# david-zwicker/video-analysis

Measured on AMD Instinct MI355X. Metric: frames/sec (bg-sub+blur+thresh+CCL) 1080p uint8, higher is better.
Workload: dtype u8; 1 GPU; cfg3_1080p_full_chain: 1920x1080 uint8, batch 256/GPU, running-mean bg-sub (f64 state) + sigma=5 Gaussian (q8.8) + threshold 20 + 5x5 dilate/erode + 4-connected labelling + object counts; inputs resident in HBM; engine=bg=1 gauss=mfma-i8(ksize=31) thresh=20 morph=2 ccl=4, video=one clip per rank, overlap=off, world_size=1, backend=single process

## Files before the change

### video-analysis_amd/csrc/va_point.hip

```cpp
#include <math.h>

#include "va_common.h"

namespace va {

namespace {

constexpr int kBlock = 256;
constexpr int kVec = 8;

__device__ __forceinline__ uint8_t sat_u8_trunc(double d)
{
    const int v = (int)d;
    return (uint8_t)(v > 255 ? 255 : v);
}

template <int V>
__global__ void __launch_bounds__(kBlock)
bg_mean_u8_kernel(const uint8_t *__restrict__ frames, uint8_t *__restrict__ diff,
                  double *__restrict__ mean, long long n_seen, int n, size_t px)
{
    size_t i0 = ((size_t)blockIdx.x * kBlock + threadIdx.x) * V;
    if (i0 >= px)
        return;
    double m[V];
#pragma unroll
    for (int k = 0; k < V; k++)
        m[k] = mean[i0 + k];
    for (int f = 0; f < n; f++) {
        uint8_t p[V];
        if (V == 8) {
            uint2 v = *reinterpret_cast<const uint2 *>(frames + (size_t)f * px + i0);
            memcpy(p, &v, 8);
        } else {
            p[0] = frames[(size_t)f * px + i0];
        }
        const double dn = (double)(n_seen + f), dn1 = (double)(n_seen + f + 1);
        uint8_t o[V];
#pragma unroll
        for (int k = 0; k < V; k++) {
            double fr = (double)p[k];
            o[k] = sat_u8_trunc(fabs(fr - m[k]));
            m[k] = m[k] * dn / dn1 + fr / dn1;
        }
        if (diff) {
            if (V == 8) {
                uint2 v;
                memcpy(&v, o, 8);
                *reinterpret_cast<uint2 *>(diff + (size_t)f * px + i0) = v;
            } else {
                diff[(size_t)f * px + i0] = o[0];
            }
        }
    }
#pragma unroll
    for (int k = 0; k < V; k++)
        mean[i0 + k] = m[k];
}

__device__ __forceinline__ double div_by_uniform(double x, double d, double y)
{
    const double q = x * y;
    const double r = fma(-q, d, x);
    return fma(r, y, q);
}

__global__ void __launch_bounds__(kBlock)
bg_reciprocals_kernel(double *__restrict__ y, long long n_seen, int n)
{
    const int f = blockIdx.x * kBlock + threadIdx.x;
    if (f < n)
        y[f] = 1.0 / (double)(n_seen + f + 1);
}

struct RecipArgs {
    double r[256];
    double lo[256];
    __device__ double operator[](int f) const { return r[f]; }
};
__device__ __forceinline__ double clear_low9(double y)
{
    return __builtin_bit_cast(double, __builtin_bit_cast(unsigned long long, y) & ~0x1FFull);
}

template <int V, typename RECIP, bool BOUNDED, bool SPLIT = false>
__global__ void __launch_bounds__(kBlock)
bg_mean_u8_fast_kernel(const uint8_t *__restrict__ frames, uint8_t *__restrict__ diff,
                       double *__restrict__ mean, const RECIP recip, long long n_seen, int n, size_t px)
{
    size_t i0 = ((size_t)blockIdx.x * kBlock + threadIdx.x) * V;
    if (i0 >= px)
        return;
    double m[V];
#pragma unroll
    for (int k = 0; k < V; k++)
        m[k] = mean[i0 + k];
    typedef unsigned int v2u __attribute__((ext_vector_type(V / 4)));
    constexpr int kAhead = 8;
    const uint8_t *src = frames + i0;
    v2u cur[kAhead], nxt[kAhead];
#pragma unroll
    for (int j = 0; j < kAhead; j++)
        nxt[j] = __builtin_nontemporal_load(
            reinterpret_cast<const v2u *>(src + (size_t)min(j, n - 1) * px));
    for (int f0 = 0; f0 < n; f0 += kAhead) {
#pragma unroll
        for (int j = 0; j < kAhead; j++)
            cur[j] = nxt[j];
        if (f0 + kAhead < n) {
#pragma unroll
            for (int j = 0; j < kAhead; j++)
                nxt[j] = __builtin_nontemporal_load(reinterpret_cast<const v2u *>(
                    src + (size_t)min(f0 + kAhead + j, n - 1) * px));
        }
#pragma unroll
        for (int j = 0; j < kAhead; j++) {
            const int f = f0 + j;
            if (f >= n)
                break;
            uint8_t p[V], o[V];
            memcpy(p, &cur[j], V);
            const double dn = (double)(n_seen + f), dn1 = (double)(n_seen + f + 1);
            const double y = recip[f];
            double yh = 0.0, yl = 0.0;
            if constexpr (SPLIT) {
                yh = clear_low9(y);
                yl = recip.lo[f];
            }
#pragma unroll
            for (int k = 0; k < V; k++) {
                const double fr = (double)p[k];
                o[k] = BOUNDED ? (uint8_t)(int)fabs(fr - m[k]) : sat_u8_trunc(fabs(fr - m[k]));
                double q2;
                if constexpr (SPLIT)
                    q2 = fma(fr, yl, fr * yh);
                else
                    q2 = div_by_uniform(fr, dn1, y);
                m[k] = div_by_uniform(m[k] * dn, dn1, y) + q2;
            }
            if (diff) {
                v2u v;
                memcpy(&v, o, V);
                __builtin_nontemporal_store(v, reinterpret_cast<v2u *>(diff + (size_t)f * px + i0));
            }
        }
    }
#pragma unroll
    for (int k = 0; k < V; k++)
        mean[i0 + k] = m[k];
}

template <int V>
__global__ void __launch_bounds__(kBlock)
bg_static_u8_kernel(const uint8_t *__restrict__ frames, uint8_t *__restrict__ diff,
                    const double *__restrict__ bg, int n, size_t px)
{
    size_t i0 = ((size_t)blockIdx.x * kBlock + threadIdx.x) * V;
    if (i0 >= px)
        return;
    double m[V];
#pragma unroll
    for (int k = 0; k < V; k++)
        m[k] = bg[i0 + k];
    for (int f = 0; f < n; f++) {
        uint8_t p[V], o[V];
        if (V == 8) {
            uint2 v = *reinterpret_cast<const uint2 *>(frames + (size_t)f * px + i0);
            memcpy(p, &v, 8);
        } else {
            p[0] = frames[(size_t)f * px + i0];
        }
#pragma unroll
        for (int k = 0; k < V; k++)
            o[k] = sat_u8_trunc(fabs((double)p[k] - m[k]));
        if (V == 8) {
            uint2 v;
            memcpy(&v, o, 8);
            *reinterpret_cast<uint2 *>(diff + (size_t)f * px + i0) = v;
        } else {
            diff[(size_t)f * px + i0] = o[0];
        }
    }
}

template <int V>
__global__ void __launch_bounds__(kBlock)
bg_ema_u8_kernel(const uint8_t *__restrict__ frames, uint8_t *__restrict__ diff,
                 float *__restrict__ bg, long long n_seen, float rate, int n, size_t px)
{
    size_t i0 = ((size_t)blockIdx.x * kBlock + threadIdx.x) * V;
    if (i0 >= px)
        return;
    float m[V];
#pragma unroll
    for (int k = 0; k < V; k++)
        m[k] = bg[i0 + k];
    for (int f = 0; f < n; f++) {
        uint8_t p[V], o[V];
        if (V == 8) {
            uint2 v = *reinterpret_cast<const uint2 *>(frames + (size_t)f * px + i0);
            memcpy(p, &v, 8);
        } else {
            p[0] = frames[(size_t)f * px + i0];
        }
        const bool first = (n_seen + f) == 0;
#pragma unroll
        for (int k = 0; k < V; k++) {
            float fr = (float)p[k];
            if (first)
                m[k] = fr;
            float d = fr - m[k];
            float a = truncf(fabsf(d));
            o[k] = (uint8_t)(int)(a > 255.0f ? 255.0f : a);
            float step = rate * d;
            m[k] = m[k] + step;
        }
        if (diff) {
            if (V == 8) {
                uint2 v;
                memcpy(&v, o, 8);
                *reinterpret_cast<uint2 *>(diff + (size_t)f * px + i0) = v;
            } else {
                diff[(size_t)f * px + i0] = o[0];
            }
        }
    }
#pragma unroll
    for (int k = 0; k < V; k++)
        bg[i0 + k] = m[k];
}

template <int V>
__global__ void __launch_bounds__(kBlock)
bg_ema_f32_kernel(const float *__restrict__ frames, float *__restrict__ diff,
                  float *__restrict__ bg, long long n_seen, float rate, int n, size_t px)
{
    size_t i0 = ((size_t)blockIdx.x * kBlock + threadIdx.x) * V;
    if (i0 >= px)
        return;
    float m[V];
#pragma unroll
    for (int k = 0; k < V; k++)
        m[k] = bg[i0 + k];
    for (int f = 0; f < n; f++) {
        float p[V], o[V];
        if (V == 4) {
            float4 v = *reinterpret_cast<const float4 *>(frames + (size_t)f * px + i0);
            p[0] = v.x, p[1] = v.y, p[2] = v.z, p[3] = v.w;
        } else {
            p[0] = frames[(size_t)f * px + i0];
        }
        const bool first = (n_seen + f) == 0;
#pragma unroll
        for (int k = 0; k < V; k++) {
            if (first)
                m[k] = p[k];
            float d = p[k] - m[k];
            o[k] = fabsf(d);
            float step = rate * d;
            m[k] = m[k] + step;
        }
        if (diff) {
            if (V == 4)
                *reinterpret_cast<float4 *>(diff + (size_t)f * px + i0) =
                    make_float4(o[0], o[1], o[2], o[3]);
            else
                diff[(size_t)f * px + i0] = o[0];
        }
    }
#pragma unroll
    for (int k = 0; k < V; k++)
        bg[i0 + k] = m[k];
}

template <int V>
__global__ void __launch_bounds__(kBlock)
welford_u8_kernel(const uint8_t *__restrict__ frames, double *__restrict__ mean,
                  double *__restrict__ m2, long long n_seen, int n, size_t px)
{
    size_t i0 = ((size_t)blockIdx.x * kBlock + threadIdx.x) * V;
    if (i0 >= px)
        return;
    double m[V], q[V];
#pragma unroll
    for (int k = 0; k < V; k++) {
        m[k] = mean[i0 + k];
        q[k] = m2[i0 + k];
    }
    for (int f = 0; f < n; f++) {
        uint8_t p[V];
        if (V == 8) {
            uint2 v = *reinterpret_cast<const uint2 *>(frames + (size_t)f * px + i0);
            memcpy(p, &v, 8);
        } else {
            p[0] = frames[(size_t)f * px + i0];
        }
        const double dn1 = (double)(n_seen + f + 1);
#pragma unroll
        for (int k = 0; k < V; k++) {
            double fr = (double)p[k];
            double delta = fr - m[k];
            m[k] = m[k] + delta / dn1;
            q[k] = q[k] + delta * (fr - m[k]);
        }
    }
#pragma unroll
    for (int k = 0; k < V; k++) {
        mean[i0 + k] = m[k];
        m2[i0 + k] = q[k];
    }
}

template <class T>
__device__ __forceinline__ double quotient_as_numpy(T v, double dn1)
{
    return (double)v / dn1;
}
template <>
__device__ __forceinline__ double quotient_as_numpy<float>(float v, double dn1)
{
    return (double)(float)((double)v / (double)(float)dn1);
}

template <class T, bool WELFORD>
__global__ void __launch_bounds__(kBlock)
temporal_stats_kernel(const T *__restrict__ frames, double *__restrict__ mean, double *__restrict__ m2,
                      long long n_seen, int n, size_t px)
{
    const size_t i = (size_t)blockIdx.x * kBlock + threadIdx.x;
    if (i >= px)
        return;
    double m = mean[i], q = WELFORD ? m2[i] : 0.0;
    for (int f = 0; f < n; f++) {
        const T v = frames[(size_t)f * px + i];
        const double dn = (double)(n_seen + f), dn1 = (double)(n_seen + f + 1);
        if (WELFORD) {
            const double fr = (double)v, delta = fr - m;
            m = m + delta / dn1;
            q = q + delta * (fr - m);
        } else {
            m = m * dn / dn1 + quotient_as_numpy<T>(v, dn1);
        }
    }
    mean[i] = m;
    if (WELFORD)
        m2[i] = q;
}

__global__ void __launch_bounds__(kBlock)
threshold_u8_kernel(const uint8_t *__restrict__ src, uint8_t *__restrict__ dst, size_t count,
                    int thresh, int maxval, int vec_ok)
{
    size_t i0 = ((size_t)blockIdx.x * kBlock + threadIdx.x) * 16;
    if (i0 >= count)
        return;
    if (vec_ok && i0 + 16 <= count) {
        uint4 v = *reinterpret_cast<const uint4 *>(src + i0);
        uint8_t p[16];
        memcpy(p, &v, 16);
#pragma unroll
        for (int k = 0; k < 16; k++)
            p[k] = (int)p[k] > thresh ? (uint8_t)maxval : (uint8_t)0;
        memcpy(&v, p, 16);
        *reinterpret_cast<uint4 *>(dst + i0) = v;
    } else {
        for (size_t i = i0; i < count && i < i0 + 16; i++)
            dst[i] = (int)src[i] > thresh ? (uint8_t)maxval : (uint8_t)0;
    }
}

__global__ void __launch_bounds__(kBlock)
time_difference_kernel(const uint8_t *__restrict__ a, const uint8_t *__restrict__ b,
                       int16_t *__restrict__ out, size_t count, int vec_ok)
{
    size_t i0 = ((size_t)blockIdx.x * kBlock + threadIdx.x) * 8;
    if (i0 >= count)
        return;
    if (vec_ok && i0 + 8 <= count) {
        uint2 va_ = *reinterpret_cast<const uint2 *>(a + i0);
        uint2 vb_ = *reinterpret_cast<const uint2 *>(b + i0);
        uint8_t pa[8], pb[8];
        int16_t o[8];
        memcpy(pa, &va_, 8);
        memcpy(pb, &vb_, 8);
#pragma unroll
        for (int k = 0; k < 8; k++)
            o[k] = (int16_t)((int)pa[k] - (int)pb[k]);
        uint4 vo;
        memcpy(&vo, o, 16);
        *reinterpret_cast<uint4 *>(out + i0) = vo;
    } else {
        for (size_t i = i0; i < count && i < i0 + 8; i++)
            out[i] = (int16_t)((int)a[i] - (int)b[i]);
    }
}

__global__ void __launch_bounds__(kBlock)
mono_mean_kernel(const uint8_t *__restrict__ src, uint8_t *__restrict__ dst, size_t pixels)
{
    size_t i = (size_t)blockIdx.x * kBlock + threadIdx.x;
    if (i >= pixels)
        return;
    double s = (double)src[3 * i] + (double)src[3 * i + 1] + (double)src[3 * i + 2];
    dst[i] = (uint8_t)(int)(s / 3.0);
}

__global__ void __launch_bounds__(kBlock)
normalize_u8_kernel(const uint8_t *__restrict__ src, uint8_t *__restrict__ dst, size_t count,
                    double fmin, double fmax, double alpha, double tmin)
{
    size_t i = (size_t)blockIdx.x * kBlock + threadIdx.x;
    if (i >= count)
        return;
    double f = (double)src[i];
    f = f < fmin ? fmin : (f > fmax ? fmax : f);
    double v = (f - fmin) * alpha + tmin;
    int iv = (int)v;
    dst[i] = (uint8_t)iv;
}

}

size_t bg_scratch_bytes(int n) { return sizeof(double) * (size_t)(n > 0 ? n : 1); }

int launch_bg(int mode, int dtype, const void *frames, void *diff, void *state, int64_t n_seen,
              double rate, int n, size_t px, hipStream_t st, double *recip_scratch, bool mean_in_u8_range)
{
    VA_REQUIRE(frames && state, "va_bg_update: frames/state must not be NULL");
    VA_REQUIRE(n >= 0 && px > 0, "va_bg_update: bad sizes n=%d px=%zu", n, px);
    if (n == 0)
        return VA_OK;
    if (dtype == VA_U8) {
        const uint8_t *fr = (const uint8_t *)frames;
        uint8_t *df = (uint8_t *)diff;
        bool vec = (px % kVec == 0) && aligned(fr, 8) && (!df || aligned(df, 8));
        int grid = vec ? cdiv((long long)(px / kVec), kBlock) : cdiv((long long)px, kBlock);
        if (mode == VA_BG_MEAN) {
            const bool wide = px % 16 == 0 && aligned(fr, 16) && (!df || aligned(df, 16));
            if (vec && n <= 256) {
                RecipArgs ra;
                for (int f = 0; f < 256; f++) {
                    const double d = (double)(n_seen + (f < n ? f : 0) + 1), y = 1.0 / d;
                    unsigned long long bits;
                    memcpy(&bits, &y, 8);
                    bits &= ~0x1FFull;
                    double yh;
                    memcpy(&yh, &bits, 8);
                    ra.r[f] = y;
                    ra.lo[f] = fma(y, fma(-d, y, 1.0), y - yh);
                }
#ifdef BG_NO_SPLIT
                const bool split = false;
#else
                const bool split = n_seen + n < (1ll << 40);
#endif
                if (wide && mean_in_u8_range && split)
                    bg_mean_u8_fast_kernel<16, RecipArgs, true, true><<<cdiv((long long)(px / 16), kBlock), kBlock, 0, st>>>(
                        fr, df, (double *)state, ra, n_seen, n, px);
                else if (wide && mean_in_u8_range)
                    bg_mean_u8_fast_kernel<16, RecipArgs, true><<<cdiv((long long)(px / 16), kBlock), kBlock, 0, st>>>(
                        fr, df, (double *)state, ra, n_seen, n, px);
                else if (wide && split)
                    bg_mean_u8_fast_kernel<16, RecipArgs, false, true><<<cdiv((long long)(px / 16), kBlock), kBlock, 0, st>>>(
                        fr, df, (double *)state, ra, n_seen, n, px);
                else if (wide)
                    bg_mean_u8_fast_kernel<16, RecipArgs, false><<<cdiv((long long)(px / 16), kBlock), kBlock, 0, st>>>(
                        fr, df, (double *)state, ra, n_seen, n, px);
                else
                    bg_mean_u8_fast_kernel<8, RecipArgs, false><<<grid, kBlock, 0, st>>>(fr, df, (double *)state, ra,
                                                                                        n_seen, n, px);
            } else if (vec && recip_scratch) {
                bg_reciprocals_kernel<<<cdiv(n, kBlock), kBlock, 0, st>>>(recip_scratch, n_seen, n);
                VA_LAUNCH_CHECK("bg_reciprocals_kernel");
                if (wide)
                    bg_mean_u8_fast_kernel<16, const double *, false><<<cdiv((long long)(px / 16), kBlock), kBlock, 0, st>>>(
                        fr, df, (double *)state, recip_scratch, n_seen, n, px);
                else
                    bg_mean_u8_fast_kernel<8, const double *, false><<<grid, kBlock, 0, st>>>(
                        fr, df, (double *)state, recip_scratch, n_seen, n, px);
            } else if (vec)
                bg_mean_u8_kernel<8><<<grid, kBlock, 0, st>>>(fr, df, (double *)state, n_seen, n, px);
            else
                bg_mean_u8_kernel<1><<<grid, kBlock, 0, st>>>(fr, df, (double *)state, n_seen, n, px);
        } else if (mode == VA_BG_EMA) {
            if (vec)
                bg_ema_u8_kernel<8><<<grid, kBlock, 0, st>>>(fr, df, (float *)state, n_seen,
                                                            (float)rate, n, px);
            else
                bg_ema_u8_kernel<1><<<grid, kBlock, 0, st>>>(fr, df, (float *)state, n_seen,
                                                            (float)rate, n, px);
        } else if (mode == VA_BG_STATIC) {
            VA_REQUIRE(df, "va_bg_update: static mode needs diff_out");
            if (vec)
                bg_static_u8_kernel<8><<<grid, kBlock, 0, st>>>(fr, df, (const double *)state, n, px);
            else
                bg_static_u8_kernel<1><<<grid, kBlock, 0, st>>>(fr, df, (const double *)state, n, px);
        } else {
            VA_REQUIRE(false, "va_bg_update: unsupported mode %d for u8 frames", mode);
        }
    } else if (dtype == VA_F32) {
        VA_REQUIRE(mode == VA_BG_EMA, "va_bg_update: float32 frames support VA_BG_EMA only");
        const float *fr = (const float *)frames;
        float *df = (float *)diff;
        bool vec = (px % 4 == 0) && aligned(fr, 16) && (!df || aligned(df, 16));
        int grid = vec ? cdiv((long long)(px / 4), kBlock) : cdiv((long long)px, kBlock);
        if (vec)
            bg_ema_f32_kernel<4><<<grid, kBlock, 0, st>>>(fr, df, (float *)state, n_seen,
                                                         (float)rate, n, px);
        else
            bg_ema_f32_kernel<1><<<grid, kBlock, 0, st>>>(fr, df, (float *)state, n_seen,
                                                         (float)rate, n, px);
    } else {
        VA_REQUIRE(false, "va_bg_update: unknown dtype %d", dtype);
    }
    VA_LAUNCH_CHECK("bg kernel");
    return VA_OK;
}

int launch_welford(const uint8_t *frames, double *mean, double *m2, int64_t n_seen, int n,
                   size_t px, hipStream_t st)
{
    VA_REQUIRE(frames && mean && m2, "va_welford_u8: NULL argument");
    if (n <= 0)
        return VA_OK;
    bool vec = (px % kVec == 0) && aligned(frames, 8);
    int grid = vec ? cdiv((long long)(px / kVec), kBlock) : cdiv((long long)px, kBlock);
    if (vec)
        welford_u8_kernel<8><<<grid, kBlock, 0, st>>>(frames, mean, m2, n_seen, n, px);
    else
        welford_u8_kernel<1><<<grid, kBlock, 0, st>>>(frames, mean, m2, n_seen, n, px);
    VA_LAUNCH_CHECK("welford_u8_kernel");
    return VA_OK;
}

int launch_temporal_stats(const void *frames, int dtype, double *mean, double *m2, int64_t n_seen, int n,
                          size_t px, hipStream_t st)
{
    VA_REQUIRE(frames && mean, "temporal statistics: NULL argument");
    VA_REQUIRE(dtype == VA_U8 || dtype == VA_I16 || dtype == VA_F32 || dtype == VA_F64,
               "temporal statistics: frames must be uint8, int16, float32 or float64 (dtype code %d)", dtype);
    if (n <= 0 || px == 0)
        return VA_OK;
    const int grid = cdiv((long long)px, kBlock);
#define VA_TS(T)                                                                                            \
    do {                                                                                                    \
        if (m2)                                                                                             \
            temporal_stats_kernel<T, true><<<grid, kBlock, 0, st>>>((const T *)frames, mean, m2, n_seen, n, px);  \
        else                                                                                                \
            temporal_stats_kernel<T, false><<<grid, kBlock, 0, st>>>((const T *)frames, mean, m2, n_seen, n, px); \
    } while (0)
    if (dtype == VA_U8)
        VA_TS(uint8_t);
    else if (dtype == VA_I16)
        VA_TS(int16_t);
    else if (dtype == VA_F32)
        VA_TS(float);
    else
        VA_TS(double);
#undef VA_TS
    VA_LAUNCH_CHECK("temporal_stats_kernel");
    return VA_OK;
}

int launch_threshold_u8(const uint8_t *src, uint8_t *dst, size_t count, int thresh, int maxval,
                        hipStream_t st)
{
    VA_REQUIRE(src && dst, "va_threshold_u8: NULL argument");
    if (count == 0)
        return VA_OK;
    int vec = aligned(src, 16) && aligned(dst, 16);
    threshold_u8_kernel<<<cdiv((long long)cdiv((long long)count, 16), kBlock), kBlock, 0, st>>>(
        src, dst, count, thresh, maxval, vec);
    VA_LAUNCH_CHECK("threshold_u8_kernel");
    return VA_OK;
}

int launch_time_difference(const uint8_t *a, const uint8_t *b, int16_t *out, size_t count,
                           hipStream_t st)
{
    VA_REQUIRE(a && b && out, "va_time_difference_u8: NULL argument");
    if (count == 0)
        return VA_OK;
    int vec = aligned(a, 8) && aligned(b, 8) && aligned(out, 16);
    time_difference_kernel<<<cdiv((long long)cdiv((long long)count, 8), kBlock), kBlock, 0, st>>>(
        a, b, out, count, vec);
    VA_LAUNCH_CHECK("time_difference_kernel");
    return VA_OK;
}

int launch_mono_mean(const uint8_t *src, uint8_t *dst, size_t pixels, hipStream_t st)
{
    VA_REQUIRE(src && dst, "va_mono_mean_u8: NULL argument");
    if (pixels == 0)
        return VA_OK;
    if (src != dst && launch_pointwise_u8_x4(src, dst, pixels, 3, 3, 0, 0.0, 0.0, 0.0, 0.0, st)) {
        VA_LAUNCH_CHECK("prepare_u8_x4_kernel");
        return VA_OK;
    }
    mono_mean_kernel<<<cdiv((long long)pixels, kBlock), kBlock, 0, st>>>(src, dst, pixels);
    VA_LAUNCH_CHECK("mono_mean_kernel");
    return VA_OK;
}

template <int C, bool SPLIT>
__global__ void __launch_bounds__(kBlock)
channel_planes_kernel(const uint8_t *__restrict__ src, uint8_t *__restrict__ dst, int h, int w, int wp,
                      size_t total_quads)
{
    const size_t t = (size_t)blockIdx.x * kBlock + threadIdx.x;
    if (t >= total_quads)
        return;
    const int qpr = wp / 4;
    const int xq = (int)(t % qpr) * 4;
    const size_t rowi = t / qpr;
    const size_t f = rowi / h, y = rowi % h;
    const uint8_t *inter_c = (SPLIT ? src : nullptr);
    uint8_t *inter = SPLIT ? nullptr : dst;
    const size_t inter_row = rowi * (size_t)w * C;
    const uint8_t *inter_any = SPLIT ? src : dst;
    if (C > 1 && xq + 3 < w && ((w * C) & 3) == 0 && (reinterpret_cast<uintptr_t>(inter_any) & 3) == 0) {
        uint32_t in[C], out[C];
        uint8_t b[4 * C], o[4 * C];
        if (SPLIT) {
#pragma unroll
            for (int c = 0; c < C; c++)
                in[c] = reinterpret_cast<const uint32_t *>(src + inter_row + (size_t)xq * C)[c];
            memcpy(b, in, 4 * C);
#pragma unroll
            for (int c = 0; c < C; c++)
                *reinterpret_cast<uint32_t *>(dst + ((f * C + c) * h + y) * (size_t)wp + xq) =
                    (uint32_t)b[c] | ((uint32_t)b[C + c] << 8) | ((uint32_t)b[2 * C + c] << 16) | ((uint32_t)b[3 * C + c] << 24);
        } else {
#pragma unroll
            for (int c = 0; c < C; c++)
                in[c] = *reinterpret_cast<const uint32_t *>(src + ((f * C + c) * h + y) * (size_t)wp + xq);
            memcpy(b, in, 4 * C);
#pragma unroll
            for (int i = 0; i < 4; i++)
#pragma unroll
                for (int c = 0; c < C; c++)
                    o[i * C + c] = b[4 * c + i];
            memcpy(out, o, 4 * C);
#pragma unroll
            for (int c = 0; c < C; c++)
                reinterpret_cast<uint32_t *>(dst + inter_row + (size_t)xq * C)[c] = out[c];
        }
        return;
    }
    if (SPLIT) {
#pragma unroll
        for (int c = 0; c < C; c++) {
            uint32_t v = 0;
#pragma unroll
            for (int i = 0; i < 4; i++) {
                int x = xq + i;
                x = x < w ? x : 2 * (w - 1) - x;
                x = max(x, 0);
                v |= (uint32_t)inter_c[inter_row + (size_t)x * C + c] << (8 * i);
            }
            *reinterpret_cast<uint32_t *>(dst + ((f * C + c) * h + y) * (size_t)wp + xq) = v;
        }
    } else {
        uint8_t p[C][4];
#pragma unroll
        for (int c = 0; c < C; c++)
            *reinterpret_cast<uint32_t *>(p[c]) =
                *reinterpret_cast<const uint32_t *>(src + ((f * C + c) * h + y) * (size_t)wp + xq);
#pragma unroll
        for (int i = 0; i < 4; i++)
            if (xq + i < w) {
#pragma unroll
                for (int c = 0; c < C; c++)
                    inter[inter_row + (size_t)(xq + i) * C + c] = p[c][i];
            }
    }
}

int launch_channel_planes(const uint8_t *src, uint8_t *dst, int n, int h, int w, int wp, int c,
                          bool split, hipStream_t st)
{
    VA_REQUIRE(src && dst && wp % 4 == 0 && wp >= w && wp - w < w && c >= 1 && c <= 4,
               "channel planes: bad arguments");
    if (n == 0)
        return VA_OK;
    const size_t total = (size_t)n * h * (wp / 4);
    const unsigned grid = (unsigned)((total + kBlock - 1) / kBlock);
#define VA_CP(CC)                                                                                   \
    do {                                                                                            \
        if (split)                                                                                  \
            channel_planes_kernel<CC, true><<<grid, kBlock, 0, st>>>(src, dst, h, w, wp, total);    \
        else                                                                                        \
            channel_planes_kernel<CC, false><<<grid, kBlock, 0, st>>>(src, dst, h, w, wp, total);   \
    } while (0)
    if (c == 1)
        VA_CP(1);
    else if (c == 2)
        VA_CP(2);
    else if (c == 3)
        VA_CP(3);
    else
        VA_CP(4);
#undef VA_CP
    VA_LAUNCH_CHECK("channel_planes_kernel");
    return VA_OK;
}

template <typename E>
__global__ void __launch_bounds__(kBlock)
rot90_kernel(const E *__restrict__ src, E *__restrict__ dst, int h, int w, int k)
{
    __shared__ E tile[32][33];
    const int ho = (k & 1) ? w : h, wo = (k & 1) ? h : w;
    const int tiles_x = (wo + 31) >> 5, tiles_y = (ho + 31) >> 5;
    int t = blockIdx.x;
    const int tx = t % tiles_x;
    t /= tiles_x;
    const int ty = t % tiles_y;
    const size_t f = t / tiles_y;
    const E *in = src + f * (size_t)h * w;
    E *out = dst + f * (size_t)h * w;
    const int lx = threadIdx.x & 31, ly = threadIdx.x >> 5;
    const int i0 = ty * 32, j0 = tx * 32;
#pragma unroll
    for (int r = 0; r < 32; r += 8) {
        const int a = ly + r, b = lx;
        int si, sj;
        if (k == 1) {
            si = j0 + a;
            sj = w - 1 - (i0 + b);
        } else if (k == 2) {
            si = h - 1 - (i0 + a);
            sj = w - 1 - (j0 + b);
        } else if (k == 3) {
            si = h - 1 - (j0 + a);
            sj = i0 + b;
        } else {
            si = i0 + a;
            sj = j0 + b;
        }
        if (si >= 0 && si < h && sj >= 0 && sj < w)
            tile[a][b] = in[(size_t)si * w + sj];
    }
    __syncthreads();
#pragma unroll
    for (int r = 0; r < 32; r += 8) {
        const int i = i0 + ly + r, j = j0 + lx;
        if (i < ho && j < wo) {
            const int di = ly + r, dj = lx;
            E v;
            if (k == 1)
                v = tile[dj][di];
            else if (k == 3)
                v = tile[dj][di];
            else
                v = tile[di][dj];
            out[(size_t)i * wo + j] = v;
        }
    }
}

struct Elem3 { uint8_t b[3]; };
struct Elem6 { uint16_t b[3]; };
struct Elem12 { uint32_t b[3]; };

int launch_rot90(const void *src, void *dst, int n, int h, int w, int elem_bytes, int k,
                 hipStream_t st)
{
    VA_REQUIRE(src && dst && src != dst, "va_rot90: src/dst must be distinct non-NULL");
    VA_REQUIRE(n >= 0 && h > 0 && w > 0, "va_rot90: bad shape (%d,%d,%d)", n, h, w);
    k &= 3;
    if (n == 0)
        return VA_OK;
    const int ho = (k & 1) ? w : h, wo = (k & 1) ? h : w;
    const size_t blocks = (size_t)n * ((ho + 31) / 32) * ((wo + 31) / 32);
    VA_REQUIRE(blocks < ((size_t)1 << 31), "va_rot90: too many tiles");
#define VA_ROT(T) rot90_kernel<T><<<(unsigned)blocks, kBlock, 0, st>>>((const T *)src, (T *)dst, h, w, k)
    switch (elem_bytes) {
    case 1: VA_ROT(uint8_t); break;
    case 2: VA_ROT(uint16_t); break;
    case 3: VA_ROT(Elem3); break;
    case 4: VA_ROT(uint32_t); break;
    case 6: VA_ROT(Elem6); break;
    case 8: VA_ROT(uint64_t); break;
    case 12: VA_ROT(Elem12); break;
    default:
        VA_REQUIRE(false, "va_rot90: unsupported pixel size of %d bytes", elem_bytes);
    }
#undef VA_ROT
    VA_LAUNCH_CHECK("rot90_kernel");
    return VA_OK;
}

int launch_normalize_u8(const uint8_t *src, uint8_t *dst, size_t count, double fmin, double fmax,
                        double alpha, double tmin, hipStream_t st)
{
    VA_REQUIRE(src && dst, "va_normalize_u8: NULL argument");
    if (count == 0)
        return VA_OK;
    if (launch_pointwise_u8_x4(src, dst, count, 1, -1, 1, fmin, fmax, alpha, tmin, st)) {
        VA_LAUNCH_CHECK("prepare_u8_x4_kernel");
        return VA_OK;
    }
    normalize_u8_kernel<<<cdiv((long long)count, kBlock), kBlock, 0, st>>>(src, dst, count, fmin,
                                                                          fmax, alpha, tmin);
    VA_LAUNCH_CHECK("normalize_u8_kernel");
    return VA_OK;
}

}
```

Measured before the change: 318,500 frames/s.

## Restructure running-mean bg kernel with ping-pong prefetch groups and compile-time diff

Rewrites the running-mean background kernel so frame loads alternate between two register groups (ping-pong), which removes the per-group register copy and the branch in the steady-state loop. It also keeps the frame counter as an incrementing double instead of converting from int64 each frame, packs diff bytes with perm instructions, and makes the diff store a template parameter. A countability guard sends extreme n_seen values to the slow path. The cost is more template instantiations and higher register pressure from holding two load groups.

```diff
diff --git a/video-analysis_amd/csrc/va_point.hip b/video-analysis_amd/csrc/va_point.hip
--- a/video-analysis_amd/csrc/va_point.hip
+++ b/video-analysis_amd/csrc/va_point.hip
@@ -83,54 +83,60 @@
     return __builtin_bit_cast(double, __builtin_bit_cast(unsigned long long, y) & ~0x1FFull);
 }
 
-template <int V, typename RECIP, bool BOUNDED, bool SPLIT = false>
-__global__ void __launch_bounds__(kBlock)
-bg_mean_u8_fast_kernel(const uint8_t *__restrict__ frames, uint8_t *__restrict__ diff,
-                       double *__restrict__ mean, const RECIP recip, long long n_seen, int n, size_t px)
-{
-    size_t i0 = ((size_t)blockIdx.x * kBlock + threadIdx.x) * V;
-    if (i0 >= px)
-        return;
-    double m[V];
-#pragma unroll
-    for (int k = 0; k < V; k++)
-        m[k] = mean[i0 + k];
-    typedef unsigned int v2u __attribute__((ext_vector_type(V / 4)));
-    constexpr int kAhead = 8;
-    const uint8_t *src = frames + i0;
-    v2u cur[kAhead], nxt[kAhead];
-#pragma unroll
-    for (int j = 0; j < kAhead; j++)
-        nxt[j] = __builtin_nontemporal_load(
-            reinterpret_cast<const v2u *>(src + (size_t)min(j, n - 1) * px));
-    for (int f0 = 0; f0 < n; f0 += kAhead) {
+__device__ __forceinline__ unsigned byte_lane(unsigned w, int k)
+{
+    return k == 3 ? w >> 24 : (w >> (8 * k)) & 0xFFu;
+}
+__device__ __forceinline__ unsigned pack_bytes(const int *d)
+{
+    const unsigned lo = __builtin_amdgcn_perm((unsigned)d[1], (unsigned)d[0], 0x0C0C0400u);
+    const unsigned hi = __builtin_amdgcn_perm((unsigned)d[3], (unsigned)d[2], 0x0C0C0400u);
+    return __builtin_amdgcn_perm(hi, lo, 0x05040100u);
+}
+
+constexpr int kAhead = 8;
+
+template <int V> struct BgGroup {
+    typedef unsigned int vec __attribute__((ext_vector_type(V / 4)));
+    vec v[kAhead];
+    template <bool CLAMP>
+    __device__ __forceinline__ void load(const uint8_t *frames, size_t i0, size_t px, int f0, int n)
+    {
 #pragma unroll
         for (int j = 0; j < kAhead; j++)
-            cur[j] = nxt[j];
-        if (f0 + kAhead < n) {
-#pragma unroll
-            for (int j = 0; j < kAhead; j++)
-                nxt[j] = __builtin_nontemporal_load(reinterpret_cast<const v2u *>(
-                    src + (size_t)min(f0 + kAhead + j, n - 1) * px));
-        }
-#pragma unroll
-        for (int j = 0; j < kAhead; j++) {
-            const int f = f0 + j;
-            if (f >= n)
-                break;
-            uint8_t p[V], o[V];
-            memcpy(p, &cur[j], V);
-            const double dn = (double)(n_seen + f), dn1 = (double)(n_seen + f + 1);
-            const double y = recip[f];
-            double yh = 0.0, yl = 0.0;
-            if constexpr (SPLIT) {
-                yh = clear_low9(y);
-                yl = recip.lo[f];
-            }
-#pragma unroll
-            for (int k = 0; k < V; k++) {
-                const double fr = (double)p[k];
-                o[k] = BOUNDED ? (uint8_t)(int)fabs(fr - m[k]) : sat_u8_trunc(fabs(fr - m[k]));
+            v[j] = __builtin_nontemporal_load(reinterpret_cast<const vec *>(
+                frames + (size_t)(CLAMP ? min(f0 + j, n - 1) : f0 + j) * px + i0));
+    }
+};
+
+template <int V, typename RECIP, bool BOUNDED, bool SPLIT, bool DIFF, bool FULL>
+__device__ __forceinline__ void bg_mean_group(const BgGroup<V> &g, double (&m)[V], double &dn, const RECIP &recip,
+                                              int f0, int cnt, uint8_t *diff, size_t i0, size_t px)
+{
+#pragma unroll
+    for (int j = 0; j < kAhead; j++) {
+        if (!FULL && j >= cnt)
+            break;
+        const int f = f0 + j;
+        const double dn1 = dn + 1.0;
+        const double y = recip[f];
+        double yh = 0.0, yl = 0.0;
+        if constexpr (SPLIT) {
+            yh = clear_low9(y);
+            yl = recip.lo[f];
+        }
+        typename BgGroup<V>::vec out;
+#pragma unroll
+        for (int w = 0; w < V / 4; w++) {
+            int d[4];
+#pragma unroll
+            for (int b = 0; b < 4; b++) {
+                const int k = 4 * w + b;
+                const double fr = (double)byte_lane(g.v[j][w], b);
+                if constexpr (DIFF) {
+                    const int a = (int)fabs(fr - m[k]);
+                    d[b] = BOUNDED ? a : min(a, 255);
+                }
                 double q2;
                 if constexpr (SPLIT)
                     q2 = fma(fr, yl, fr * yh);
@@ -138,12 +144,44 @@
                     q2 = div_by_uniform(fr, dn1, y);
                 m[k] = div_by_uniform(m[k] * dn, dn1, y) + q2;
             }
-            if (diff) {
-                v2u v;
-                memcpy(&v, o, V);
-                __builtin_nontemporal_store(v, reinterpret_cast<v2u *>(diff + (size_t)f * px + i0));
-            }
-        }
+            if constexpr (DIFF)
+                out[w] = pack_bytes(d);
+        }
+        if constexpr (DIFF)
+            __builtin_nontemporal_store(out, reinterpret_cast<typename BgGroup<V>::vec *>(diff + (size_t)f * px + i0));
+        dn = dn1;
+    }
+}
+
+template <int V, typename RECIP, bool BOUNDED, bool SPLIT, bool DIFF>
+__global__ void __launch_bounds__(kBlock)
+bg_mean_u8_fast_kernel(const uint8_t *__restrict__ frames, uint8_t *__restrict__ diff,
+                       double *__restrict__ mean, const RECIP recip, double dn0, int n, size_t px)
+{
+    const size_t i0 = ((size_t)blockIdx.x * kBlock + threadIdx.x) * V;
+    if (i0 >= px)
+        return;
+    double m[V];
+#pragma unroll
+    for (int k = 0; k < V; k++)
+        m[k] = mean[i0 + k];
+    double dn = dn0;
+    BgGroup<V> a, b;
+    a.template load<true>(frames, i0, px, 0, n);
+    int f0 = 0;
+    for (; f0 + 3 * kAhead <= n; f0 += 2 * kAhead) {
+        b.template load<false>(frames, i0, px, f0 + kAhead, n);
+        bg_mean_group<V, RECIP, BOUNDED, SPLIT, DIFF, true>(a, m, dn, recip, f0, kAhead, diff, i0, px);
+        a.template load<false>(frames, i0, px, f0 + 2 * kAhead, n);
+        bg_mean_group<V, RECIP, BOUNDED, SPLIT, DIFF, true>(b, m, dn, recip, f0 + kAhead, kAhead, diff, i0, px);
+    }
+    for (; f0 < n; f0 += kAhead) {
+        const bool more = f0 + kAhead < n;
+        if (more)
+            b.template load<true>(frames, i0, px, f0 + kAhead, n);
+        bg_mean_group<V, RECIP, BOUNDED, SPLIT, DIFF, false>(a, m, dn, recip, f0, min(kAhead, n - f0), diff, i0, px);
+        if (more)
+            a = b;
     }
 #pragma unroll
     for (int k = 0; k < V; k++)
@@ -421,6 +459,19 @@
 
 }
 
+template <int V, typename RECIP, bool BOUNDED, bool SPLIT>
+static void launch_bg_fast(const uint8_t *fr, uint8_t *df, double *mean, const RECIP &recip, double dn0, int n,
+                           size_t px, hipStream_t st)
+{
+    const int grid = cdiv((long long)(px / V), kBlock);
+    if constexpr (BOUNDED)
+        bg_mean_u8_fast_kernel<V, RECIP, true, SPLIT, true><<<grid, kBlock, 0, st>>>(fr, df, mean, recip, dn0, n, px);
+    else if (df)
+        bg_mean_u8_fast_kernel<V, RECIP, BOUNDED, SPLIT, true><<<grid, kBlock, 0, st>>>(fr, df, mean, recip, dn0, n, px);
+    else
+        bg_mean_u8_fast_kernel<V, RECIP, BOUNDED, SPLIT, false><<<grid, kBlock, 0, st>>>(fr, df, mean, recip, dn0, n, px);
+}
+
 size_t bg_scratch_bytes(int n) { return sizeof(double) * (size_t)(n > 0 ? n : 1); }
 
 int launch_bg(int mode, int dtype, const void *frames, void *diff, void *state, int64_t n_seen,
@@ -437,7 +488,11 @@
         int grid = vec ? cdiv((long long)(px / kVec), kBlock) : cdiv((long long)px, kBlock);
         if (mode == VA_BG_MEAN) {
             const bool wide = px % 16 == 0 && aligned(fr, 16) && (!df || aligned(df, 16));
-            if (vec && n <= 256) {
+            const bool countable = n_seen >= -(1ll << 53) && n_seen <= (1ll << 53) - n;
+            const bool bounded = mean_in_u8_range && df;
+            const double dn0 = (double)n_seen;
+            double *mean = (double *)state;
+            if (vec && countable && n <= 256) {
                 RecipArgs ra;
                 for (int f = 0; f < 256; f++) {
                     const double d = (double)(n_seen + (f < n ? f : 0) + 1), y = 1.0 / d;
@@ -454,30 +509,23 @@
 #else
                 const bool split = n_seen + n < (1ll << 40);
 #endif
-                if (wide && mean_in_u8_range && split)
-                    bg_mean_u8_fast_kernel<16, RecipArgs, true, true><<<cdiv((long long)(px / 16), kBlock), kBlock, 0, st>>>(
-                        fr, df, (double *)state, ra, n_seen, n, px);
-                else if (wide && mean_in_u8_range)
-                    bg_mean_u8_fast_kernel<16, RecipArgs, true><<<cdiv((long long)(px / 16), kBlock), kBlock, 0, st>>>(
-                        fr, df, (double *)state, ra, n_seen, n, px);
+                if (wide && bounded && split)
+                    launch_bg_fast<16, RecipArgs, true, true>(fr, df, mean, ra, dn0, n, px, st);
+                else if (wide && bounded)
+                    launch_bg_fast<16, RecipArgs, true, false>(fr, df, mean, ra, dn0, n, px, st);
                 else if (wide && split)
-                    bg_mean_u8_fast_kernel<16, RecipArgs, false, true><<<cdiv((long long)(px / 16), kBlock), kBlock, 0, st>>>(
-                        fr, df, (double *)state, ra, n_seen, n, px);
+                    launch_bg_fast<16, RecipArgs, false, true>(fr, df, mean, ra, dn0, n, px, st);
                 else if (wide)
-                    bg_mean_u8_fast_kernel<16, RecipArgs, false><<<cdiv((long long)(px / 16), kBlock), kBlock, 0, st>>>(
-                        fr, df, (double *)state, ra, n_seen, n, px);
+                    launch_bg_fast<16, RecipArgs, false, false>(fr, df, mean, ra, dn0, n, px, st);
                 else
-                    bg_mean_u8_fast_kernel<8, RecipArgs, false><<<grid, kBlock, 0, st>>>(fr, df, (double *)state, ra,
-                                                                                        n_seen, n, px);
-            } else if (vec && recip_scratch) {
+                    launch_bg_fast<8, RecipArgs, false, false>(fr, df, mean, ra, dn0, n, px, st);
+            } else if (vec && countable && recip_scratch) {
                 bg_reciprocals_kernel<<<cdiv(n, kBlock), kBlock, 0, st>>>(recip_scratch, n_seen, n);
                 VA_LAUNCH_CHECK("bg_reciprocals_kernel");
                 if (wide)
-                    bg_mean_u8_fast_kernel<16, const double *, false><<<cdiv((long long)(px / 16), kBlock), kBlock, 0, st>>>(
-                        fr, df, (double *)state, recip_scratch, n_seen, n, px);
+                    launch_bg_fast<16, const double *, false, false>(fr, df, mean, recip_scratch, dn0, n, px, st);
                 else
-                    bg_mean_u8_fast_kernel<8, const double *, false><<<grid, kBlock, 0, st>>>(
-                        fr, df, (double *)state, recip_scratch, n_seen, n, px);
+                    launch_bg_fast<8, const double *, false, false>(fr, df, mean, recip_scratch, dn0, n, px, st);
             } else if (vec)
                 bg_mean_u8_kernel<8><<<grid, kBlock, 0, st>>>(fr, df, (double *)state, n_seen, n, px);
             else
```

Measured after the change: 323,500 frames/s (median of 6 runs). +1.5%, better.
